# MasatoAkiyama/jama16-retina-replication

Hardware: AMD Instinct MI355X
Metric: train images/sec, Inception-v3 299^2 bs64/GPU (higher is better)
Workload: dtype f32; 1 GPU; Inception-v3 299x299 f32 training, batch 64/GPU, Nesterov lr 3e-3 m 0.9; model=inception_v3, global_batch=64, parallelism=dp1, ranks=1, hip_graph=False, lanes=2, tiles=pinned

## Files before the change

### include/jr.h

```cpp
#ifndef JR_H_
#define JR_H_

#include <stddef.h>
#include <stdint.h>

#ifdef __cplusplus
extern "C" {
#endif

typedef enum jr_status {
  JR_OK = 0,
  JR_ERR_INVALID = -1,
  JR_ERR_HIP = -2,
  JR_ERR_UNSUPPORTED = -3,
  JR_ERR_WORKSPACE = -4,
  JR_ERR_DEVICE = -5
} jr_status;

typedef enum jr_dtype { JR_F32 = 0, JR_BF16 = 1, JR_F32_X8 = 2, JR_F32_X8P = 3, JR_F32_X6H = 4 } jr_dtype;

typedef enum jr_conv_op { JR_CONV_FWD = 0, JR_CONV_BWD_DATA = 1, JR_CONV_BWD_FILTER = 2 } jr_conv_op;

typedef enum jr_head_mode { JR_HEAD_SIGMOID = 0, JR_HEAD_SOFTMAX = 1 } jr_head_mode;

// ... 44 lines not shown
int jr_conv2d_fwd_bn_partials(const jr_conv_desc* d, int dtype, const void* x, const void* w, void* y, void* ws,
                              size_t ws_bytes, void* stream);
int jr_conv2d_bwd_data(const jr_conv_desc* d, int dtype, const void* dy, const void* w, void* dx,
                       int accumulate, void* ws, size_t ws_bytes, void* stream);
int jr_conv2d_bwd_filter(const jr_conv_desc* d, int dtype, const void* x, const void* dy, float* dw,
                         void* ws, size_t ws_bytes, void* stream);

typedef struct jr_wgrad_seg {
  const float* slabs;
  float* dw;
  int32_t m, n, splits, c_in, c_pad, g, block0, blocks;
} jr_wgrad_seg;
int jr_conv2d_wgrad_seg(const jr_conv_desc* d, int dtype, jr_wgrad_seg* seg);
int jr_conv2d_bwd_filter_slabs(const jr_conv_desc* d, int dtype, const void* x, const void* dy, float* slabs,
                               size_t slab_bytes, void* stream);
int jr_wgrad_reduce(const jr_wgrad_seg* segs, int32_t nseg, int32_t total_blocks, void* stream);

int jr_conv2d_autotune(const jr_conv_desc* d, int op, int dtype, const void* a, const void* b, void* c,
                       void* ws, size_t ws_bytes, void* stream);
int jr_conv2d_get_config(const jr_conv_desc* d, int op, int dtype, int phase);
int jr_conv2d_set_config(const jr_conv_desc* d, int op, int dtype, int phase, int cfg);
int jr_conv2d_num_configs(int dtype);
unsigned long long jr_conv2d_config_generation(void);

size_t jr_bn_workspace_size(int64_t m, int32_t c);
typedef struct jr_bn_launch_plan {
  int32_t vec_width, rows_per_chunk, nchunks, single_stage;
  int32_t reduce_grid, finalize_grid, stats_finalize_grid, apply_grid;
  int32_t fold_rows, fold_grid_x, fold_grid_y, reserved;
  int64_t k1_offset, workspace_size;
} jr_bn_launch_plan;
int jr_bn_plan(int dtype, int64_t m, int32_t c, jr_bn_launch_plan* out);
int jr_bn_stats(int dtype, const void* x, int64_t m, int32_t c, float eps, float* mean, float* invstd,
                void* ws, size_t ws_bytes, void* stream);
int jr_bn_relu_apply(int dtype, const void* x, int32_t x_c_off, int32_t x_c_stride, int64_t m, int32_t c,
                     const float* mean, const float* invstd, const float* beta, void* y, int32_t y_c_off,
                     int32_t y_c_stride, void* stream);
typedef struct jr_bn_apply_seg {
  void* y;
  int32_t y_c_off, y_c_stride, c;
  const float* beta;
} jr_bn_apply_seg;
int jr_bn_relu_apply_multi(int dtype, int nseg, const jr_bn_apply_seg* segs, const void* x, int32_t x_c_off,
                           int32_t x_c_stride, int64_t m, int32_t c, const float* mean, const float* invstd,
                           void* stream);
int jr_bn_relu_apply_stats(int dtype, const void* x, int32_t x_c_off, int32_t x_c_stride, int64_t m, int32_t c,
// ... 167 lines not shown
```

### jama16-retina-replication_amd/csrc/jr_common.h

```cpp
#pragma once
#include <hip/hip_runtime.h>
#include <hip/hip_bf16.h>
#include <stdint.h>
#include <cstdlib>
#include <string>

#include "jr_bn_plan.h"
#include "jr_error.h"

namespace jr {

int check_launch(const char* what);

inline hipStream_t as_stream(void* s) { return reinterpret_cast<hipStream_t>(s); }

unsigned* stream_scratch(hipStream_t s, int kind, size_t words);

unsigned* device_error_word(hipStream_t s);

__device__ __forceinline__ int xcd_remap(int orig, int nwg) {
  const int xcd = orig & 7;
  const int q = nwg >> 3, r = nwg & 7;
  const int base = xcd < r ? xcd * (q + 1) : r * (q + 1) + (xcd - r) * q;
  return base + (orig >> 3);
}

__device__ __forceinline__ float bf2f(uint16_t v) {
  return __uint_as_float(static_cast<uint32_t>(v) << 16);
}
__device__ __forceinline__ uint16_t f2bf(float f) {
  __hip_bfloat16 h = __float2bfloat16(f);
  return *reinterpret_cast<uint16_t*>(&h);
}

__device__ __forceinline__ float bn_xhat(float x, float mean, float invstd) {
  return __fmul_rn(__fsub_rn(x, mean), invstd);
}
__device__ __forceinline__ float bn_pre(float x, float mean, float invstd, float beta) {
  return __fadd_rn(bn_xhat(x, mean, invstd), beta);
}

__device__ __forceinline__ void stats_combine8(const float* __restrict__ pm, const float* __restrict__ pq, int P,
                                               int R, int M, float eps, int j, float* mean, float* invstd) {
  const double K = pm[0];
  double sn = 0, sd = 0, sq = 0;
  constexpr int U = 16;
  for (int i0 = j; i0 < P; i0 += kStatsLanes * U) {
    float vm[U], vq[U];
// ... 57 lines not shown
```

### jama16-retina-replication_amd/csrc/jr_conv.hip

```cpp
#include "jr_conv_loop.h"

#include <algorithm>
#include <type_traits>
#include <vector>

namespace jr {

__device__ __forceinline__ uint32_t pk_bf16(float a, float b) {
  const bf16x2 r = {(__bf16)a, (__bf16)b};
  return __builtin_bit_cast(uint32_t, r);
}

__device__ __forceinline__ float sub_f32(float a, float b) {
  float r;
  asm("v_sub_f32 %0, %1, %2" : "=v"(r) : "v"(a), "v"(b));
  return r;
}

__device__ __forceinline__ float lo_bf16_f32(uint32_t u) {
  uint32_t r;
  asm("v_lshlrev_b32 %0, 16, %1" : "=v"(r) : "v"(u));
  return __uint_as_float(r);
}

// ... 70 lines not shown
    }
#pragma unroll
    for (int p = 0; p < 4; ++p) lp[p] = pkrtz_f16(x[2 * p], x[2 * p + 1]);
  }
  typedef uint32_t u32x4 __attribute__((ext_vector_type(4)));
  __device__ __forceinline__ f16x8 h() const { return __builtin_bit_cast(f16x8, (u32x4){hp[0], hp[1], hp[2], hp[3]}); }
  __device__ __forceinline__ f16x8 m() const { return __builtin_bit_cast(f16x8, (u32x4){mp[0], mp[1], mp[2], mp[3]}); }
  __device__ __forceinline__ f16x8 l() const { return __builtin_bit_cast(f16x8, (u32x4){lp[0], lp[1], lp[2], lp[3]}); }
};

template <int OP, int BM, int BN, int WGM, int BK, int NBUF, bool UT, bool X8, int DBG = 0, bool SK = false,
          bool H6 = false>
__global__ void __launch_bounds__(256) k_conv(ConvArgs g) {
  using G = TileGeom<BM, BN, WGM, 4, BK, 4>;
  constexpr int WGN = G::WGN, WM = G::WM, WN = G::WN, TM = G::TM, TN = G::TN;
  constexpr int QPR = G::QPR, RPI = G::RPI, SWZ = G::SWZ, ASZ = G::ASZ, BSZ = G::BSZ;
  constexpr int A_INSTR = G::A_INSTR, B_INSTR = G::B_INSTR, A_PW = G::A_PW, B_PW = G::B_PW;
  constexpr int HALF = BK / 2;
  constexpr bool A_KC = (OP != OP_WGRAD);
  constexpr bool B_KC = (OP == OP_DGRAD);
  constexpr int SMEM = NBUF * (ASZ + BSZ) > 4 * stage_floats<WN>() ? NBUF * (ASZ + BSZ) : 4 * stage_floats<WN>();
  __shared__ __attribute__((aligned(1024))) float smem[SMEM];
  JR_ST(Stamps stamp; stamp.start();)
  member_offsets(g);

  const int tid = threadIdx.x;
  const int lane = tid & 63;
  const int wave = __builtin_amdgcn_readfirstlane(tid >> 6);
  float h_sa = 1.f, h_sb = 1.f, h_one = 1.f;
  if constexpr (H6) {
    asm volatile("" : "+s"(h_one));
    h_sa = __uint_as_float(__builtin_amdgcn_readfirstlane(
        __float_as_uint(pow2_scale(g.a_max ? absmax64(g.a_max, lane) : g.a_bnd))));
    h_sb = __uint_as_float(__builtin_amdgcn_readfirstlane(
        __float_as_uint(pow2_scale(g.b_max ? absmax64(g.b_max, lane) : g.b_bnd))));
  }
  const int wm0 = (wave / WGN) * WM;
  const int wn0 = (wave % WGN) * WN;

  long long sk_it = 0, sk_end = 0;
  const int lb = SK ? xcd_remap(blockIdx.x, gridDim.x) : 0;
  if constexpr (SK) {
    const long long W = (long long)((g.M + BM - 1) / BM) * g.ntn * g.ktiles;
    sk_it = (long long)lb * g.sk_ipb;
    sk_end = sk_it + g.sk_ipb < W ? sk_it + g.sk_ipb : W;
  }
  bool sk_first = true;
  for (;;) {
  int tile, kt0, kt1;
  if constexpr (SK) {
    if (sk_it >= sk_end) break;
    tile = (int)(sk_it / g.ktiles);
    kt0 = (int)(sk_it - (long long)tile * g.ktiles);
    kt1 = (int)(sk_end - sk_it < (long long)(g.ktiles - kt0) ? kt0 + (sk_end - sk_it) : g.ktiles);
    sk_it += kt1 - kt0;
    if (!sk_first) __syncthreads();
  } else {
    tile = xcd_remap(blockIdx.x, gridDim.x);
    kt0 = blockIdx.z * g.kt_per_split;
    kt1 = min(g.ktiles, kt0 + g.kt_per_split);
  }
  const int mt = tile / g.ntn, nt = tile - mt * g.ntn;
  const int m0 = mt * BM, n0 = nt * BN;
  const float* zp = g_zero_page;
  const int cred = OP == OP_FWD ? g.cp : g.cout;
  constexpr bool ut = UT && OP != OP_WGRAD;
  const int wq = OP == OP_WGRAD ? BK / g.wo : 0, wr = OP == OP_WGRAD ? BK - wq * g.wo : 0;
  const int dW0 = OP == OP_WGRAD ? (wq * g.sh * g.w + wr * g.sw) * g.xs : 0;
  const int dW1 = OP == OP_WGRAD ? (g.sh * g.w - g.wo * g.sw) * g.xs : 0;
  const int dW2 = OP == OP_WGRAD ? (g.h * g.w - g.ho * g.sh * g.w) * g.xs : 0;

  const float* a_ptr[A_PW];
  int a_p0[A_PW], a_p1[A_PW], a_p2[A_PW];
  int a_s0[A_PW], a_s1[A_PW], a_s2[A_PW];
  int a_off[A_PW];
#pragma unroll
  for (int i = 0; i < A_PW; ++i) {
    const int j = wave + 4 * i;
    a_ptr[i] = zp;
    a_p0[i] = a_p1[i] = a_p2[i] = 0;
    a_s0[i] = a_s1[i] = a_s2[i] = 0;
    a_off[i] = 0;
// ... 528 lines not shown
    if (rc) return rc;
    hipLaunchKernelGGL(k_stats_finalize, dim3(N, 1, members), dim3(256), 0, s, (const float*)s2,
                       (const float*)(s2 + 2 * (size_t)N * S), S, 0, M, N, S, st->eps, st->mean, st->invstd,
                       (float*)nullptr, pm, st_mb);
  }
  return check_launch("conv stats finalize");
}

static int run_conv1_direct(const jr_conv_desc* d, int dtype, const void* x, const void* w, void* y, void* ws,
                            size_t ws_bytes, hipStream_t s, const StatsReq* st, int members = 1, long long x_mb = 0,
                            long long w_mb = 0, long long y_mb = 0, long long st_mb = 0) {
  int P, R;
  conv1_direct_partials(d, &P, &R);
  const size_t wsm = conv1_direct_ws(d);
  if (st && (!ws || ws_bytes < wsm * members)) return fail(JR_ERR_WORKSPACE, "conv1 direct: workspace too small");
  float* stats = st ? static_cast<float*>(ws) : nullptr;
  launch_conv1_direct(d, dtype, x, w, y, stats, members, x_mb, w_mb, y_mb, (long long)wsm, s);
  int rc = check_launch("conv1 direct");
  if (rc || !st) return rc;
  const long long M = (long long)d->n * d->ho * d->wo;
  return finalize_stats(stats, P, R, (int)M, d->c_out, members, (long long)wsm, st, st_mb, s);
}

template <int OP>
static int run_gemm(int dtype, ConvArgs a, const Plan& p, void* out, void* ws, size_t ws_bytes, hipStream_t s,
                    const StatsReq* st = nullptr, bool defer = false, int members = 1, long long st_mb = 0) {
  if (p.M <= 0 || p.N <= 0) return JR_OK;
  const size_t wsm = members > 1 ? member_ws(dtype, p, st != nullptr) : 0;
  if (members > 1 && (!ws || ws_bytes < wsm * members) && (p.splits > 1 || st))
    return fail(JR_ERR_WORKSPACE, "conv grouped: workspace too small (jr_conv2d_workspace_size_grouped)");
  int sP = 0, sR = 0;
  if (st) {
    stats_geom(dtype, p, &sP, &sR);
    const size_t off = align256(plan_ws(p));
    if (!ws || ws_bytes < off + stats_ws(dtype, p)) return fail(JR_ERR_WORKSPACE, "conv: workspace too small for BN statistics");
    a.stats = reinterpret_cast<float*>(static_cast<char*>(ws) + off);
    a.stats_p = sP;
    a.s_mb = (long long)wsm;
  }
  a.M = p.M; a.N = p.N; a.K = p.K;
  JR_ST(a.dbg = g_dbg_stamps;)
  a.ktiles = p.ktiles;
  a.kt_per_split = p.kt_per_split;
  a.ntn = p.nt;
  a.slab_elems = (long long)p.M * p.N;
  if (p.splits > 1) {
    if (!ws || ws_bytes < plan_ws(p)) return fail(JR_ERR_WORKSPACE, "conv: workspace too small for split-K");
    a.C = static_cast<float*>(ws);
    a.c_mb = (long long)wsm;
  } else {
    a.C = static_cast<float*>(out);
    a.c_mb = a.o_mb;
  }
  dim3 grid(p.mt * p.nt, members, p.splits);
  if (p.sk) {
    if (!ws || ws_bytes < plan_ws(p) + (members > 1 ? (size_t)(members - 1) * wsm : 0))
      return fail(JR_ERR_WORKSPACE, "conv: workspace too small for the stream-K hand-off");
    a.sk_ipb = p.sk_ipb;
    a.sk_part = static_cast<float*>(ws);
    a.sk_mb = (long long)wsm;
    a.sk_flags = stream_scratch(s, 0, (size_t)p.sk_blocks * members);
    if (!a.sk_flags) return fail(JR_ERR_HIP, "conv: stream-K flag words could not be allocated");
    a.sk_fmb = (long long)p.sk_blocks * sizeof(unsigned);
    a.sk_err = device_error_word(s);
    if (!a.sk_err) return fail(JR_ERR_HIP, "conv: no device error word (call jr_init before capturing)");
    grid = dim3(p.sk_blocks, members, 1);
  }
  const CfgEntry& e = cfg_entry(dtype, p.tile);
  switch (e.kernel) {
    case Kernel::HALO:
      a.halo_wp = a.w + a.kw - 1;
      a.halo_nr = (e.t->bm + a.wo - 2) / a.wo + 1 + a.kh - 1;
      launch_conv_halo(e.index, a, grid, s);
      break;
    case Kernel::BF16:
    case Kernel::BF16_WIDE: {
      const TileCfg& t = *e.t;
      int am;
      if (OP == OP_WGRAD) {
        am = t.bk / a.wo < a.ho ? 1 : 2;
      } else {
        const int cred = OP == OP_FWD ? a.cp : a.cout;
        am = cred % t.bk == 0 ? 0 : cred >= t.bk ? 1 : 2;
      }
      const bool wide = e.kernel == Kernel::BF16_WIDE;
      const int np = dtype == JR_F32_X8P ? 3 : 1;
      if (e.sk) launch_conv_bf16_sk(OP, e.index, wide, am, a, grid, s);
      else if (wide) launch_conv_bf16_wide(OP, e.index, am, a, grid, s, np);
      else launch_conv_bf16(OP, e.index, am, a, grid, s, np);
// ... 404 lines not shown
  return autotune(d, op, dtype, a, b, c, ws, ws_bytes, stream, 3);
}

JR_API int jr_conv2d_num_configs(int dtype) { return cfg_count(dtype); }

JR_API int jr_conv2d_debug_time(const jr_conv_desc* d, int cfg, int dbg, const void* x, const void* w, void* y,
                                int reps, float* ms, void* stream) {
  int rc = validate(d, OP_FWD, JR_F32);
  if (rc) return rc;
  const bool x8 = dbg >= 16;
  if (x8) dbg -= 16;
  if (cfg < 0 || cfg >= kNumCfgs || dbg < 0 || dbg > (x8 ? 4 : 3)) return fail(JR_ERR_INVALID, "debug_time: bad cfg/dbg");
  if (dbg > 0 && chan_pad(d->c_in, JR_F32) % kCfgs[cfg].bk != 0)
    return fail(JR_ERR_UNSUPPORTED, "debug_time: variants need c_in % BK == 0");
  ConvArgs a = conv_args(d, OP_FWD, JR_F32, x, w);
  a.C = (float*)y;
  Plan p = plan_for(d, OP_FWD, JR_F32, Phase{}, cfg);
  p.splits = 1; p.kt_per_split = p.ktiles;
  a.M = p.M; a.N = p.N; a.K = p.K; a.ktiles = p.ktiles; a.kt_per_split = p.kt_per_split; a.ntn = p.nt;
  hipStream_t s = as_stream(stream);
  hipEvent_t e0, e1;
  (void)hipEventCreate(&e0);
  (void)hipEventCreate(&e1);
  dim3 grid(p.mt * p.nt, 1, 1);
  (void)hipEventRecord(e0, s);
  for (int r = 0; r < reps; ++r) {
    switch (dbg + (x8 ? 16 : 0)) {
      case 0: launch_op<OP_FWD, 0>(cfg, a, grid, s); break;
      case 1: launch_op<OP_FWD, 1>(cfg, a, grid, s); break;
      case 2: launch_op<OP_FWD, 2>(cfg, a, grid, s); break;
      case 3: launch_op<OP_FWD, 3>(cfg, a, grid, s); break;
      case 16: launch_op<OP_FWD, 0, true>(cfg, a, grid, s); break;
      case 17: launch_op<OP_FWD, 1, true>(cfg, a, grid, s); break;
      case 18: launch_op<OP_FWD, 2, true>(cfg, a, grid, s); break;
      case 19: launch_op<OP_FWD, 3, true>(cfg, a, grid, s); break;
      default: launch_op<OP_FWD, 4, true>(cfg, a, grid, s); break;
    }
  }
  (void)hipEventRecord(e1, s);
  (void)hipEventSynchronize(e1);
  (void)hipEventElapsedTime(ms, e0, e1);
  (void)hipEventDestroy(e0);
  (void)hipEventDestroy(e1);
  return check_launch("debug_time");
}

JR_API int jr_conv2d_set_config(const jr_conv_desc* d, int op, int dtype, int phase, int cfg) {
// ... 22 lines not shown
```

### jama16-retina-replication_amd/csrc/jr_conv_bf16.hip

```cpp
#include "jr_conv_loop.h"

namespace jr {

__device__ __forceinline__ s16x4 lds_tr(const uint16_t* p) {
  return __builtin_amdgcn_ds_read_tr16_b64_v4i16(
      (__attribute__((address_space(3))) s16x4*)(const_cast<uint16_t*>(p)));
}

template <int OP, int BM, int BN, int WGM, int BK, int NBUF, int AM, int NP, int NW, bool SK = false>
__global__ void __launch_bounds__(NW * 64) k_conv_bf16(ConvArgs g) {
  static_assert(NP == 1 || NP == 3, "one bf16 plane, or the h / m / l planes of X8P");
  static_assert(NW == 4 || NW == 8, "4 or 8 waves per block");
  using G = TileGeom<BM, BN, WGM, NW, BK, 8>;
  constexpr int WGN = G::WGN, WM = G::WM, WN = G::WN, TM = G::TM, TN = G::TN;
  constexpr int QPR = G::QPR, RPI = G::RPI, SWZ = G::SWZ, ASZ = G::ASZ, BSZ = G::BSZ;
  constexpr int A_INSTR = G::A_INSTR, B_INSTR = G::B_INSTR, A_PW = G::A_PW, B_PW = G::B_PW;
  constexpr int KSTEPS = BK / 16;
  constexpr bool MC = (OP == OP_WGRAD);
  static_assert(BK % 16 == 0 && QPR <= 8, "BK must be 16..64");
  constexpr int STAGE = NP * (ASZ + BSZ);
  constexpr int SMEM = NBUF * STAGE > 2 * NW * stage_floats<WN>() ? NBUF * STAGE : 2 * NW * stage_floats<WN>();
  static_assert(SMEM * 2 <= 160 * 1024, "LDS budget of one CU");
  __shared__ __attribute__((aligned(1024))) uint16_t smem[SMEM];

  JR_ST(Stamps stamp; stamp.start();)
  member_offsets(g);
  const uint16_t* __restrict__ gA = reinterpret_cast<const uint16_t*>(g.A);
  const uint16_t* __restrict__ gB = reinterpret_cast<const uint16_t*>(g.B);
  const int tid = threadIdx.x;
  const int lane = tid & 63;
  const int wave = __builtin_amdgcn_readfirstlane(tid >> 6);
  const int wm0 = (wave / WGN) * WM;
  const int wn0 = (wave % WGN) * WN;

  long long sk_it = 0, sk_end = 0;
  const int lb = SK ? xcd_remap(blockIdx.x, gridDim.x) : 0;
  if constexpr (SK) {
    const long long W = (long long)((g.M + BM - 1) / BM) * g.ntn * g.ktiles;
    sk_it = (long long)lb * g.sk_ipb;
    sk_end = sk_it + g.sk_ipb < W ? sk_it + g.sk_ipb : W;
  }
  bool sk_first = true;
  for (;;) {
  int tile, kt0, kt1;
  if constexpr (SK) {
    if (sk_it >= sk_end) break;
    tile = (int)(sk_it / g.ktiles);
    kt0 = (int)(sk_it - (long long)tile * g.ktiles);
    kt1 = (int)(sk_end - sk_it < (long long)(g.ktiles - kt0) ? kt0 + (sk_end - sk_it) : g.ktiles);
    sk_it += kt1 - kt0;
    if (!sk_first) __syncthreads();
  } else {
    tile = xcd_remap(blockIdx.x, gridDim.x);
    kt0 = blockIdx.z * g.kt_per_split;
    kt1 = min(g.ktiles, kt0 + g.kt_per_split);
  }
  const int mt = tile / g.ntn, nt = tile - mt * g.ntn;
  const int m0 = mt * BM, n0 = nt * BN;
  unsigned long long zpa = reinterpret_cast<unsigned long long>(g_zero_page);
  asm volatile("" : "+s"(zpa));
  const uint16_t* zp = reinterpret_cast<const uint16_t*>(zpa);
  const int cred = OP == OP_FWD ? g.cp : g.cout;
  const long long psA = NP > 1 ? g.a_ps : 0, psB = NP > 1 ? g.b_ps : 0;
  constexpr bool ut = AM == 0 && OP != OP_WGRAD;

  const int wq = OP == OP_WGRAD ? BK / g.wo : 0, wr = OP == OP_WGRAD ? BK - wq * g.wo : 0;
  constexpr bool inc_a = AM == 1;
  constexpr bool inc_b = OP == OP_DGRAD && AM == 1;
  const int dA0 = OP == OP_WGRAD ? (wq * g.sh * g.w + wr * g.sw) * g.xs : BK;
  const int dA1 = OP == OP_FWD ? BK - g.cp + g.xs
                  : OP == OP_DGRAD ? BK - g.cout - g.ys
                                   : (g.sh * g.w - g.wo * g.sw) * g.xs;
  const int dA2 = OP == OP_FWD ? BK - g.cp + g.xs + (g.w - g.kw) * g.xs
                  : OP == OP_DGRAD ? BK - g.cout + (g.nb - 1 - g.wo) * g.ys
                                   : (g.h * g.w - g.ho * g.sh * g.w) * g.xs;
  const int dB1 = OP == OP_DGRAD ? BK - g.cout + g.sw * g.cin * g.cout : 0;
  const int dB2 = OP == OP_DGRAD ? BK - g.cout + (g.sh * g.kw - g.sw * (g.nb - 1)) * g.cin * g.cout : 0;
// ... 458 lines not shown
```

### jama16-retina-replication_amd/csrc/jr_conv_halo.hip

```cpp
#include "jr_conv_loop.h"

namespace jr {

template <int KH, int KW, int BM, int BN, int WGM, int NBUF, int SLOTS>
__global__ void __launch_bounds__(256) k_conv_halo(ConvArgs g) {
  constexpr int BK = 32;
  constexpr int TAPS = KH * KW;
  using G = WaveTile<BM, BN, WGM, 4>;
  constexpr int WGN = G::WGN, WM = G::WM, WN = G::WN, TM = G::TM, TN = G::TN;
  static_assert(SLOTS % 16 == 0 && (TAPS * BN) % 16 == 0, "images must be whole DMA instructions");
  constexpr int A_INSTR = SLOTS / 16, B_INSTR = TAPS * BN / 16;
  constexpr int A_PW = (A_INSTR + 3) / 4, B_PW = (B_INSTR + 3) / 4;
  constexpr int ASZ = SLOTS * BK, BSZ = TAPS * BN * BK;
  constexpr int STAGE = ASZ + BSZ;
  constexpr int SMEM = NBUF * STAGE > 8 * stage_floats<WN>() ? NBUF * STAGE : 8 * stage_floats<WN>();
  __shared__ __attribute__((aligned(1024))) uint16_t smem[SMEM];
  constexpr int NPIECE = A_PW + B_PW;
  constexpr int per_tile = A_INSTR / 4 + B_INSTR / 4;
  constexpr int KSTEPS = 2 * TAPS;

  member_offsets(g);
  const uint16_t* __restrict__ gA = reinterpret_cast<const uint16_t*>(g.A);
  const uint16_t* __restrict__ gB = reinterpret_cast<const uint16_t*>(g.B);
  const int tid = threadIdx.x;
  const int lane = tid & 63;
  const int wave = __builtin_amdgcn_readfirstlane(tid >> 6);
  const int wm0 = (wave / WGN) * WM;
  const int wn0 = (wave % WGN) * WN;
  const int tile = xcd_remap(blockIdx.x, gridDim.x);
  const int mt = tile / g.ntn, nt = tile - mt * g.ntn;
  const int m0 = mt * BM, n0 = nt * BN;
  const int kt0 = blockIdx.z * g.kt_per_split;
  const int kt1 = min(g.ktiles, kt0 + g.kt_per_split);
  const uint16_t* zp = reinterpret_cast<const uint16_t*>(g_zero_page);
  const int WP = g.halo_wp;
  const int gr0 = m0 / g.wo;
  const int glo = gr0 - g.ph;
  const int nslots = g.halo_nr * WP;
  const int grows = g.n * g.h;

  const uint16_t* a_ptr[A_PW];
#pragma unroll
  for (int i = 0; i < A_PW; ++i) {
    const int j = wave + 4 * i;
    a_ptr[i] = nullptr;
    if (A_INSTR % 4 != 0 && j >= A_INSTR) continue;
    const int e = j * 64 + lane;
    const int s = e >> 2, q = (e & 3) ^ ((s >> 2) & 3);
    if (s < nslots) {
      const int sr = s / WP, sc = s - sr * WP;
      const int G = glo + sr, iw = sc - g.pw;
      if ((unsigned)G < (unsigned)grows && (unsigned)iw < (unsigned)g.w)
        a_ptr[i] = gA + (((long long)G * g.w + iw) * g.xs + g.xo + q * 8);
    }
  }
// ... 141 lines not shown
```

### jama16-retina-replication_amd/csrc/jr_conv_impl.h

```cpp
#pragma once
#include "jr_common.h"
#include "jr_conv_plan.h"

#include <type_traits>

namespace jr {

typedef float f32x16 __attribute__((ext_vector_type(16)));

static __device__ __attribute__((aligned(64))) float g_zero_page[16];

struct ConvArgs {
  const float* A;
  const float* B;
  float* C;
  int M, N, K;
  int n, h, w, cin, cp, cout, kh, kw, sh, sw, ph, pw, ho, wo;
  int xo, xs, yo, ys;
  int c_off, c_stride;
  int accumulate;
  int ktiles, kt_per_split, ntn;
  long long slab_elems;
  float* stats;
  int stats_p;
  int py, px, r0, c0, na, nb, ey, ex, hc, wc;
  long long a_ps, b_ps;
  int halo_nr, halo_wp;
  unsigned long long* dbg;
  long long a_mb, b_mb, c_mb, s_mb, o_mb;
  long long sk_ipb, sk_mb, sk_fmb;
  unsigned* sk_flags;
  float* sk_part;
  unsigned* sk_err;
  const float* a_max;
  const float* b_max;
  float a_bnd, b_bnd;
};

__device__ __forceinline__ float absmax64(const float* p, int lane) {
  float v = p[lane];
#pragma unroll
  for (int o = 32; o >= 1; o >>= 1) v = fmaxf(v, __shfl_xor(v, o, 64));
  return v;
}

__device__ __forceinline__ float pow2_scale(float m) {
  const unsigned b = __float_as_uint(m);
  const int eb = (int)((b >> 23) & 0xffu);
  if (!(m > 0.f) || eb == 255) return 1.f;
  const int biased = min(268 - eb, 227);
  return __uint_as_float((unsigned)biased << 23);
}

__device__ __forceinline__ void member_offsets(ConvArgs& g) {
  if (gridDim.y > 1) {
    const long long m = blockIdx.y;
    g.A = reinterpret_cast<const float*>(reinterpret_cast<const char*>(g.A) + m * g.a_mb);
    g.B = reinterpret_cast<const float*>(reinterpret_cast<const char*>(g.B) + m * g.b_mb);
    g.C = reinterpret_cast<float*>(reinterpret_cast<char*>(g.C) + m * g.c_mb);
    if (g.stats) g.stats = reinterpret_cast<float*>(reinterpret_cast<char*>(g.stats) + m * g.s_mb);
    if (g.a_max) g.a_max += 64 * m;
    if (g.b_max) g.b_max += 64 * m;
    if (g.sk_flags) {
      g.sk_flags = reinterpret_cast<unsigned*>(reinterpret_cast<char*>(g.sk_flags) + m * g.sk_fmb);
      g.sk_part = reinterpret_cast<float*>(reinterpret_cast<char*>(g.sk_part) + m * g.sk_mb);
    }
  }
}

#ifdef JR_STAMPS
struct Stamps {
  unsigned long long r0, c0, cp, cl, w;
  __device__ __forceinline__ void start() {
    r0 = __builtin_amdgcn_s_memrealtime();
    c0 = __builtin_amdgcn_s_memtime();
    w = 0;
  }
  __device__ __forceinline__ void prologue() { cp = __builtin_amdgcn_s_memtime(); }
  __device__ __forceinline__ void loop() { cl = __builtin_amdgcn_s_memtime(); }
  __device__ __forceinline__ unsigned long long now() { return __builtin_amdgcn_s_memtime(); }
  __device__ __forceinline__ void end(unsigned long long* dbg) {
    const unsigned long long ce = __builtin_amdgcn_s_memtime(), re = __builtin_amdgcn_s_memrealtime();
    if (dbg == nullptr || threadIdx.x != 0) return;
    unsigned long long* o = dbg + 8ull * (blockIdx.z * gridDim.x + blockIdx.x);
    o[0] = r0; o[1] = re; o[2] = cp - c0; o[3] = cl - cp; o[4] = ce - cl; o[5] = w;
    o[6] = __builtin_amdgcn_s_getreg((31 << 11) | 4);
    o[7] = __builtin_amdgcn_s_getreg((3 << 11) | 20);
  }
};
#define JR_ST(x) x
#else
#define JR_ST(x)
#endif

__device__ __forceinline__ long long dgrad_pix(const ConvArgs& g, int m) {
  const int hw = g.hc * g.wc;
  const int b = m / hw, rem = m - b * hw;
  const int u = rem / g.wc, v = rem - u * g.wc;
  return ((long long)b * g.h + g.sh * u + g.py) * g.w + g.sw * v + g.px;
}

template <int OP>
__device__ __forceinline__ long long out_row(const ConvArgs& g, int m) {
  if constexpr (OP == OP_FWD) {
    return (long long)m * g.c_stride + g.c_off;
  } else if constexpr (OP == OP_DGRAD) {
    return dgrad_pix(g, m) * g.c_stride + g.c_off;
// ... 155 lines not shown
  }
  sk_sum_pieces<TM, TN, NW>(g, acc, wave, lane, owner, npieces, st == 2);
  return true;
}

__device__ __forceinline__ bool sk_cut(const ConvArgs& g, int tile, int kt0, int kt1, int* owner, int* npieces,
                                       int* kind) {
  if (kt0 == 0 && kt1 == g.ktiles) return false;
  const long long t0 = (long long)tile * g.ktiles;
  *owner = (int)(t0 / g.sk_ipb);
  *npieces = (int)((t0 + g.ktiles - 1) / g.sk_ipb) - *owner + 1;
  *kind = kt0 == 0 ? 1 : 0;
  return true;
}


template <int WN> constexpr int stage_floats() { return 32 * (WN + 8); }

template <int OP, int WM, int TM, int TN, bool BF16K>
__device__ __forceinline__ void conv_epilogue(const ConvArgs& g, f32x16 (&acc)[TM][TN], float* stage, int mw0,
                                              int nw0, int lane) {
  constexpr int WN = TN * 32, S = WN + 8, LPR = WN / 8, NIT = 32 * LPR / 64;
  static_assert((32 * LPR) % 64 == 0, "stage read-back must be whole wave-instructions");
  const bool split = gridDim.z > 1;
  const bool bout = BF16K && OP != OP_WGRAD && !split;
  const int l31 = lane & 31, lh = lane >> 5;
  auto row_of = [&](int r) { return (r & 3) + 8 * (r >> 2) + 4 * lh; };
  if constexpr (OP == OP_FWD) {
    if (g.stats != nullptr && !split) {
      const int P = g.stats_p;
      const int pidx = mw0 / WM;
      const int nv = min(max(g.M - mw0, 0), WM);
#pragma unroll
      for (int j = 0; j < TN; ++j) {
        float s = 0.f;
#pragma unroll
        for (int i = 0; i < TM; ++i)
#pragma unroll
          for (int r = 0; r < 16; ++r) {
            float v = acc[i][j][r];
            if (bout) { v = bf2f(f2bf(v)); acc[i][j][r] = v; }
            s += (mw0 + i * 32 + row_of(r) < g.M) ? v : 0.f;
          }
        s += __shfl_xor(s, 32, 64);
        const float mu = nv > 0 ? s / (float)nv : 0.f;
        float q = 0.f;
#pragma unroll
        for (int i = 0; i < TM; ++i)
#pragma unroll
          for (int r = 0; r < 16; ++r) {
            const float d = acc[i][j][r] - mu;
            q += (mw0 + i * 32 + row_of(r) < g.M) ? d * d : 0.f;
          }
        q += __shfl_xor(q, 32, 64);
        const int n = nw0 + j * 32 + l31;
        if (lh == 0 && n < g.N) {
          g.stats[(long long)n * P + pidx] = mu;
          g.stats[(long long)(g.N + n) * P + pidx] = q;
        }
      }
    }
  }
  float* C = split ? g.C + (long long)blockIdx.z * g.slab_elems : g.C;
#pragma unroll
  for (int i = 0; i < TM; ++i) {
#pragma unroll
    for (int j = 0; j < TN; ++j)
#pragma unroll
      for (int r = 0; r < 16; ++r) stage[row_of(r) * S + j * 32 + l31] = acc[i][j][r];
    asm volatile("s_waitcnt lgkmcnt(0)" ::: "memory");
    constexpr int CH = NIT % 4 == 0 ? 4 : NIT % 3 == 0 ? 3 : NIT % 2 == 0 ? 2 : 1;
#pragma unroll
    for (int i0 = 0; i0 < NIT; i0 += CH) {
      float v[CH][8];
      long long off[CH];
      bool ok[CH];
#pragma unroll
      for (int k = 0; k < CH; ++k) {
        const int e = (i0 + k) * 64 + lane;
        const int row = e / LPR, c8 = (e - row * LPR) * 8;
        const float4 v0 = *reinterpret_cast<const float4*>(stage + row * S + c8);
        const float4 v1 = *reinterpret_cast<const float4*>(stage + row * S + c8 + 4);
        v[k][0] = v0.x; v[k][1] = v0.y; v[k][2] = v0.z; v[k][3] = v0.w;
        v[k][4] = v1.x; v[k][5] = v1.y; v[k][6] = v1.z; v[k][7] = v1.w;
        const int m = mw0 + i * 32 + row, n = nw0 + c8;
        ok[k] = m < g.M && n < g.N;
// ... 233 lines not shown
```

### jama16-retina-replication_amd/csrc/jr_conv_plan.cpp

```cpp
#include "jr_conv_plan.h"

#include <algorithm>
#include <cstdlib>
#include <map>
#include <mutex>
#include <vector>

namespace jr {

struct CfgSpace {
  std::vector<CfgEntry> ids;
  int std;
};

static CfgSpace build_space(int dtype) {
  CfgSpace s;
  auto tiles = [&](Kernel k, const TileCfg* t, int n, bool sk) {
    for (int i = 0; i < n; ++i) s.ids.push_back(CfgEntry{k, i, sk, t + i, nullptr});
  };
  switch (dtype) {
    case JR_F32:
      tiles(Kernel::F32_MFMA, kCfgs, kNumCfgs, false);
      s.std = kNumCfgs;
      break;
    case JR_F32_X8:
// ... 295 lines not shown
  std::lock_guard<std::mutex> lk(c.mu);
  auto it = c.tuned.find(k);
  return it != c.tuned.end() ? it->second : -1;
}

void tune_set(const TuneKey& k, int cfg) {
  TuneCache& c = tune_cache();
  std::lock_guard<std::mutex> lk(c.mu);
  auto it = c.tuned.find(k);
  if (cfg < 0) {
    if (it != c.tuned.end()) { c.tuned.erase(it); ++c.gen; }
  } else if (it == c.tuned.end() || it->second != cfg) {
    c.tuned[k] = cfg;
    ++c.gen;
  }
}

unsigned long long tune_generation() {
  TuneCache& c = tune_cache();
  std::lock_guard<std::mutex> lk(c.mu);
  return c.gen;
}

}
```

### jama16-retina-replication_amd/csrc/jr_conv_plan.h

```cpp
#pragma once
#include <array>
#include <cstddef>

#include "jr_error.h"

namespace jr {

enum { OP_FWD = 0, OP_DGRAD = 1, OP_WGRAD = 2 };

inline size_t align256(size_t b) { return (b + 255) / 256 * 256; }

#ifndef JR_STATS_CHUNK
#define JR_STATS_CHUNK 4096
#endif
constexpr int kStatsChunk = JR_STATS_CHUNK;

struct TileCfg {
  int bm, bn, wgm, bk, nbuf;
  double eff;
  int nw = 4;
};

static constexpr TileCfg kCfgs[] = {
    {128, 128, 2, 16, 3, 1.00},
    {128, 128, 2, 32, 2, 1.00},
    {256, 64, 4, 16, 3, 1.00},
// ... 166 lines not shown
```

### jama16-retina-replication_amd/jr/_ffi.py

```python
from __future__ import annotations

import ctypes
import os
from ctypes import (POINTER, Structure, c_char_p, c_double, c_float, c_int, c_int32, c_int64,
                    c_size_t, c_uint8, c_void_p)

_HERE = os.path.dirname(os.path.abspath(__file__))
LIB_PATH = os.environ.get("JR_LIB", os.path.join(_HERE, "libjr.so"))

JR_OK = 0
JR_ERR_INVALID, JR_ERR_HIP, JR_ERR_UNSUPPORTED, JR_ERR_WORKSPACE = -1, -2, -3, -4
JR_ERR_DEVICE = -5
JR_F32 = 0
JR_BF16 = 1
JR_F32_X8 = 2
JR_F32_X8P = 3
JR_F32_X6H = 4
JR_CONV_FWD, JR_CONV_BWD_DATA, JR_CONV_BWD_FILTER = 0, 1, 2
JR_HEAD_SIGMOID, JR_HEAD_SOFTMAX = 0, 1


class JRError(RuntimeError):

    def __init__(self, fn: str, status: int, msg: str):
# ... 79 lines not shown
    "jr_conv2d_fwd_bn_partials": (c_int, [POINTER(ConvDesc), c_int, c_void_p, c_void_p, c_void_p, c_void_p, c_size_t,
                                          c_void_p]),
    "jr_bn_relu_apply_stats": (c_int, [c_int, c_void_p, c_int32, c_int32, c_int64, c_int32, c_void_p, c_int32, c_int32,
                                       c_int32, c_int32, c_float, c_void_p, c_void_p, c_void_p, c_void_p, c_int32,
                                       c_int32, c_void_p]),
    "jr_conv2d_workspace_size_grouped": (c_size_t, [POINTER(ConvDesc), c_int, c_int]),
    "jr_conv2d_fwd_bn_stats_grouped": (c_int, [POINTER(ConvDesc), c_int, c_int, c_void_p, c_int64, c_void_p, c_int64,
                                               c_void_p, c_int64, c_float, c_void_p, c_void_p, c_int64, c_void_p,
                                               c_size_t, c_void_p]),
    "jr_conv2d_bwd_data": (c_int, [POINTER(ConvDesc), c_int, c_void_p, c_void_p, c_void_p, c_int,
                                   c_void_p, c_size_t, c_void_p]),
    "jr_conv2d_bwd_filter": (c_int, [POINTER(ConvDesc), c_int, c_void_p, c_void_p, c_void_p,
                                     c_void_p, c_size_t, c_void_p]),
    "jr_conv2d_wgrad_seg": (c_int, [POINTER(ConvDesc), c_int, POINTER(WgradSeg)]),
    "jr_conv2d_bwd_filter_slabs": (c_int, [POINTER(ConvDesc), c_int, c_void_p, c_void_p, c_void_p, c_size_t,
                                           c_void_p]),
    "jr_wgrad_reduce": (c_int, [c_void_p, c_int32, c_int32, c_void_p]),
    "jr_conv2d_autotune": (c_int, [POINTER(ConvDesc), c_int, c_int, c_void_p, c_void_p, c_void_p,
                                   c_void_p, c_size_t, c_void_p]),
    "jr_conv2d_get_config": (c_int, [POINTER(ConvDesc), c_int, c_int, c_int]),
    "jr_conv2d_set_config": (c_int, [POINTER(ConvDesc), c_int, c_int, c_int, c_int]),
    "jr_conv2d_config_generation": (ctypes.c_ulonglong, []),
    "jr_conv2d_num_configs": (c_int, [c_int]),
    "jr_conv_weights_bf16_tiles": (c_int32, [c_int32, c_int32, c_int32, c_int32]),
    "jr_conv_weights_bf16": (c_int, [c_void_p, c_int32, c_int32, c_int32, c_int32, c_void_p, c_void_p,
                                     c_void_p]),
    "jr_conv_weights_bf16_multi": (c_int, [c_void_p, c_int32, c_int32, c_void_p, c_void_p, c_void_p,
                                           c_void_p]),
    "jr_conv_weights_x8p": (c_int, [c_void_p, c_int32, c_int32, c_int32, c_int32, c_void_p, c_void_p,
                                    c_void_p]),
    "jr_conv_weights_x8p_multi": (c_int, [c_void_p, c_int32, c_int32, c_void_p, c_void_p, c_void_p,
                                          c_void_p]),
    "jr_split_x8p": (c_int, [c_void_p, c_int64, c_int32, c_int32, c_int32, c_void_p, c_int32, c_int32, c_int32,
                             c_int64, c_void_p]),
    "jr_comm_unique_id": (c_int, [c_void_p]),
    "jr_comm_init": (c_int, [c_int, c_int, c_void_p, c_int, c_void_p]),
    "jr_comm_init_file": (c_int, [c_int, c_int, c_char_p, c_char_p, c_int, c_int, c_void_p]),
    "jr_allreduce_sum": (c_int, [c_void_p, c_void_p, c_size_t, c_int, c_void_p]),
    "jr_comm_rank": (c_int, [c_void_p]),
    "jr_comm_world": (c_int, [c_void_p]),
    "jr_comm_destroy": (c_int, [c_void_p]),
    "jr_bn_workspace_size": (c_size_t, [c_int64, c_int32]),
    "jr_bn_plan": (c_int, [c_int, c_int64, c_int32, POINTER(BnLaunchPlan)]),
    "jr_bn_relu_bwd_batch_workspace_size": (c_size_t, [c_int32, c_void_p]),
    "jr_bn_relu_apply_multi": (c_int, [c_int, c_int, c_void_p, c_void_p, c_int32, c_int32, c_int64, c_int32,
                                       c_void_p, c_void_p, c_void_p]),
# ... 177 lines not shown
```

### jama16-retina-replication_amd/jr/engine.py

```python
from __future__ import annotations

import ctypes
import dataclasses
import json
import os
from typing import Callable, Dict, List, Optional, Tuple

import numpy as np
import torch

from . import _ffi
from .inception import BN_EPS, Graph, PoolNode, build_inception_v3
from .init import init_params
from .lanes import Build, Call, Lanes, node_lanes, schedule
from .plan import ConvUnit, bn_batch_groups, bn_moving_segments, build_plan

DTYPES = {"f32": _ffi.JR_F32, "bf16": _ffi.JR_BF16}


_PINNED = None


def fusable_pools(g: Graph, plan) -> Dict[int, int]:
    out = {}
# ... 155 lines not shown
            self.labels[:y.numel()].copy_(y, non_blocking=True)

    def _check_images(self, images, B: int) -> None:
        ib = self.g.bufs[self.g.input_buf]
        if B > self.batch or B <= 0:
            raise ValueError(f"batch {B} outside 1..{self.batch}")
        if tuple(images.shape[1:]) != (ib.h, ib.w, ib.c):
            raise ValueError(f"images must be [B,{ib.h},{ib.w},{ib.c}] NHWC, got {tuple(images.shape)}")

    def _alloc_bn_moving(self) -> None:
        self.moving = self._t(self.members * self.stats_ms)
        self.frozen = self._t(self.members * self.stats_ms)
        self._bn_tables: Dict[int, tuple] = {}
        self._reset_bn_moving()
        self.frozen_source = None
        self.updates = 0

    def _reset_bn_moving(self, var: float = 1.0) -> None:
        host = np.zeros((self.members, self.stats_ms), np.float32)
        off = 0
        for u in self.cunits:
            host[:, off + u.cout:off + 2 * u.cout] = var
            off += 2 * u.cout
        with torch.cuda.stream(self.stream):
            self.moving.copy_(torch.from_numpy(host.reshape(-1)).to(self.device))

    def _bn_table(self, B: int) -> tuple:
        if B not in self._bn_tables:
            segs = [_ffi.BnMovingSeg(so, mo, rows, c, 0) for so, mo, rows, c in bn_moving_segments(self.cunits, B)]
            self._bn_tables[B] = (self._table(_ffi.BnMovingSeg, segs), len(segs), max(u.cout for u in self.cunits))
        return self._bn_tables[B]

    def _bn_update_args(self, B: int, momentum: float, s) -> tuple:
        table, nseg, max_c = self._bn_table(B)
        return (table.data_ptr(), nseg, max_c, self.members, self.stats.data_ptr(), self.stats_ms,
                self.moving.data_ptr(), self.stats_ms, float(momentum), BN_EPS, s)

    def _bn_layers(self):
        off = 0
        for u in self.cunits:
            for n, co in zip(u.members, u.col_off):
                yield n, off + co, off + u.cout + co
            off += 2 * u.cout

    def _bn_moving_get(self) -> List[dict]:
        self.synchronize()
# ... 892 lines not shown
```

Before: 3029 images/sec.

## Flatten conv grid and apply XCD remap across tiles, members and splits

Conv kernels now launch a 1-D grid by default and decode each block's tile, member and split index through one global XCD remap, replacing the per-tile remap on a 3-D grid. The goal is to place blocks that share operands (same member or split) on the same XCD so they reuse its L2. Decoding uses a magic-number divide, the split slab offset moves into the block setup, and an env var or API call can restore the old order. The cost is a little extra index arithmetic per block, and it may scatter tiles that previously shared data within an XCD.

```diff
diff --git a/include/jr.h b/include/jr.h
--- a/include/jr.h
+++ b/include/jr.h
@@ -90,6 +90,9 @@
 int jr_conv2d_set_config(const jr_conv_desc* d, int op, int dtype, int phase, int cfg);
 int jr_conv2d_num_configs(int dtype);
 unsigned long long jr_conv2d_config_generation(void);
+int jr_conv2d_get_block_order(void);
+int jr_conv2d_set_block_order(int order);
+int jr_conv2d_block_map(int order, int ntiles, int members, int splits, int32_t* out);
 
 size_t jr_bn_workspace_size(int64_t m, int32_t c);
 typedef struct jr_bn_launch_plan {
diff --git a/jama16-retina-replication_amd/csrc/jr_block_order.h b/jama16-retina-replication_amd/csrc/jr_block_order.h
--- /dev/null
+++ b/jama16-retina-replication_amd/csrc/jr_block_order.h
@@ -0,0 +1,44 @@
+#pragma once
+
+#if defined(__HIP__)
+#define JR_HD __attribute__((host)) __attribute__((device)) inline __attribute__((always_inline))
+#else
+#define JR_HD inline
+#endif
+
+namespace jr {
+
+JR_HD int xcd_remap(int orig, int nwg) {
+  const int xcd = orig & 7;
+  const int q = nwg >> 3, r = nwg & 7;
+  const int base = xcd < r ? xcd * (q + 1) : r * (q + 1) + (xcd - r) * q;
+  return base + (orig >> 3);
+}
+
+struct BlockPos {
+  int tile, member, split;
+};
+
+JR_HD BlockPos conv_block_pos(int order, int id, int ntiles, int members, int splits, unsigned magic) {
+  const int l = order ? xcd_remap(id, ntiles * members * splits) : id;
+  int ms = 0;
+  if (members * splits > 1)
+    ms = magic ? (int)(((unsigned long long)(unsigned)l * magic) >> 32) : ntiles == 1 ? l : (int)((unsigned)l / (unsigned)ntiles);
+  const int t = l - ms * ntiles;
+  const int s = members > 1 ? (int)((unsigned)ms / (unsigned)members) : ms;
+  return BlockPos{order ? t : xcd_remap(t, ntiles), ms - s * members, s};
+}
+
+JR_HD unsigned div_magic(int d, long long n) {
+  if (d <= 1 || (unsigned long long)n * (unsigned)d > (1ull << 32)) return 0;
+  return (unsigned)(((1ull << 32) + (unsigned)d - 1) / (unsigned)d);
+}
+
+JR_HD BlockPos conv_block_pos(int order, int id, int ntiles, int members, int splits) {
+  return conv_block_pos(order, id, ntiles, members, splits, div_magic(ntiles, (long long)ntiles * members * splits));
+}
+
+int conv_block_order();
+int set_conv_block_order(int order);
+
+}
diff --git a/jama16-retina-replication_amd/csrc/jr_common.h b/jama16-retina-replication_amd/csrc/jr_common.h
--- a/jama16-retina-replication_amd/csrc/jr_common.h
+++ b/jama16-retina-replication_amd/csrc/jr_common.h
@@ -5,6 +5,7 @@
 #include <cstdlib>
 #include <string>
 
+#include "jr_block_order.h"
 #include "jr_bn_plan.h"
 #include "jr_error.h"
 
@@ -18,12 +19,6 @@
 
 unsigned* device_error_word(hipStream_t s);
 
-__device__ __forceinline__ int xcd_remap(int orig, int nwg) {
-  const int xcd = orig & 7;
-  const int q = nwg >> 3, r = nwg & 7;
-  const int base = xcd < r ? xcd * (q + 1) : r * (q + 1) + (xcd - r) * q;
-  return base + (orig >> 3);
-}
 
 __device__ __forceinline__ float bf2f(uint16_t v) {
   return __uint_as_float(static_cast<uint32_t>(v) << 16);
diff --git a/jama16-retina-replication_amd/csrc/jr_conv.hip b/jama16-retina-replication_amd/csrc/jr_conv.hip
--- a/jama16-retina-replication_amd/csrc/jr_conv.hip
+++ b/jama16-retina-replication_amd/csrc/jr_conv.hip
@@ -116,7 +116,8 @@
   constexpr int SMEM = NBUF * (ASZ + BSZ) > 4 * stage_floats<WN>() ? NBUF * (ASZ + BSZ) : 4 * stage_floats<WN>();
   __shared__ __attribute__((aligned(1024))) float smem[SMEM];
   JR_ST(Stamps stamp; stamp.start();)
-  member_offsets(g);
+  const BlockPos bp = conv_block<SK>(g);
+  block_offsets(g, bp);
 
   const int tid = threadIdx.x;
   const int lane = tid & 63;
@@ -150,8 +151,8 @@
     sk_it += kt1 - kt0;
     if (!sk_first) __syncthreads();
   } else {
-    tile = xcd_remap(blockIdx.x, gridDim.x);
-    kt0 = blockIdx.z * g.kt_per_split;
+    tile = bp.tile;
+    kt0 = bp.split * g.kt_per_split;
     kt1 = min(g.ktiles, kt0 + g.kt_per_split);
   }
   const int mt = tile / g.ntn, nt = tile - mt * g.ntn;
@@ -726,6 +727,13 @@
   return finalize_stats(stats, P, R, (int)M, d->c_out, members, (long long)wsm, st, st_mb, s);
 }
 
+static dim3 conv_grid(ConvArgs& a, int tiles, int members, int splits) {
+  a.b_tiles = tiles; a.b_members = members; a.b_splits = splits;
+  a.b_order = conv_block_order();
+  a.b_magic = div_magic(tiles, (long long)tiles * members * splits);
+  return a.b_order ? dim3(tiles * members * splits) : dim3(tiles, members, splits);
+}
+
 template <int OP>
 static int run_gemm(int dtype, ConvArgs a, const Plan& p, void* out, void* ws, size_t ws_bytes, hipStream_t s,
                     const StatsReq* st = nullptr, bool defer = false, int members = 1, long long st_mb = 0) {
@@ -756,7 +764,8 @@
     a.C = static_cast<float*>(out);
     a.c_mb = a.o_mb;
   }
-  dim3 grid(p.mt * p.nt, members, p.splits);
+  if ((long long)p.mt * p.nt * members * p.splits > 0x7fffffffLL) return fail(JR_ERR_UNSUPPORTED, "conv: too many blocks");
+  dim3 grid = conv_grid(a, p.mt * p.nt, members, p.splits);
   if (p.sk) {
     if (!ws || ws_bytes < plan_ws(p) + (members > 1 ? (size_t)(members - 1) * wsm : 0))
       return fail(JR_ERR_WORKSPACE, "conv: workspace too small for the stream-K hand-off");
@@ -769,6 +778,7 @@
     a.sk_err = device_error_word(s);
     if (!a.sk_err) return fail(JR_ERR_HIP, "conv: no device error word (call jr_init before capturing)");
     grid = dim3(p.sk_blocks, members, 1);
+    a.b_tiles = p.sk_blocks; a.b_members = members; a.b_splits = 1; a.b_order = 0;
   }
   const CfgEntry& e = cfg_entry(dtype, p.tile);
   switch (e.kernel) {
@@ -1219,7 +1229,7 @@
   hipEvent_t e0, e1;
   (void)hipEventCreate(&e0);
   (void)hipEventCreate(&e1);
-  dim3 grid(p.mt * p.nt, 1, 1);
+  const dim3 grid = conv_grid(a, p.mt * p.nt, 1, 1);
   (void)hipEventRecord(e0, s);
   for (int r = 0; r < reps; ++r) {
     switch (dbg + (x8 ? 16 : 0)) {
diff --git a/jama16-retina-replication_amd/csrc/jr_conv_bf16.hip b/jama16-retina-replication_amd/csrc/jr_conv_bf16.hip
--- a/jama16-retina-replication_amd/csrc/jr_conv_bf16.hip
+++ b/jama16-retina-replication_amd/csrc/jr_conv_bf16.hip
@@ -24,7 +24,8 @@
   __shared__ __attribute__((aligned(1024))) uint16_t smem[SMEM];
 
   JR_ST(Stamps stamp; stamp.start();)
-  member_offsets(g);
+  const BlockPos bp = conv_block<SK>(g);
+  block_offsets(g, bp);
   const uint16_t* __restrict__ gA = reinterpret_cast<const uint16_t*>(g.A);
   const uint16_t* __restrict__ gB = reinterpret_cast<const uint16_t*>(g.B);
   const int tid = threadIdx.x;
@@ -51,8 +52,8 @@
     sk_it += kt1 - kt0;
     if (!sk_first) __syncthreads();
   } else {
-    tile = xcd_remap(blockIdx.x, gridDim.x);
-    kt0 = blockIdx.z * g.kt_per_split;
+    tile = bp.tile;
+    kt0 = bp.split * g.kt_per_split;
     kt1 = min(g.ktiles, kt0 + g.kt_per_split);
   }
   const int mt = tile / g.ntn, nt = tile - mt * g.ntn;
diff --git a/jama16-retina-replication_amd/csrc/jr_conv_halo.hip b/jama16-retina-replication_amd/csrc/jr_conv_halo.hip
--- a/jama16-retina-replication_amd/csrc/jr_conv_halo.hip
+++ b/jama16-retina-replication_amd/csrc/jr_conv_halo.hip
@@ -19,7 +19,8 @@
   constexpr int per_tile = A_INSTR / 4 + B_INSTR / 4;
   constexpr int KSTEPS = 2 * TAPS;
 
-  member_offsets(g);
+  const BlockPos bp = conv_block<false>(g);
+  block_offsets(g, bp);
   const uint16_t* __restrict__ gA = reinterpret_cast<const uint16_t*>(g.A);
   const uint16_t* __restrict__ gB = reinterpret_cast<const uint16_t*>(g.B);
   const int tid = threadIdx.x;
@@ -27,10 +28,10 @@
   const int wave = __builtin_amdgcn_readfirstlane(tid >> 6);
   const int wm0 = (wave / WGN) * WM;
   const int wn0 = (wave % WGN) * WN;
-  const int tile = xcd_remap(blockIdx.x, gridDim.x);
+  const int tile = bp.tile;
   const int mt = tile / g.ntn, nt = tile - mt * g.ntn;
   const int m0 = mt * BM, n0 = nt * BN;
-  const int kt0 = blockIdx.z * g.kt_per_split;
+  const int kt0 = bp.split * g.kt_per_split;
   const int kt1 = min(g.ktiles, kt0 + g.kt_per_split);
   const uint16_t* zp = reinterpret_cast<const uint16_t*>(g_zero_page);
   const int WP = g.halo_wp;
diff --git a/jama16-retina-replication_amd/csrc/jr_conv_impl.h b/jama16-retina-replication_amd/csrc/jr_conv_impl.h
--- a/jama16-retina-replication_amd/csrc/jr_conv_impl.h
+++ b/jama16-retina-replication_amd/csrc/jr_conv_impl.h
@@ -28,6 +28,8 @@
   int halo_nr, halo_wp;
   unsigned long long* dbg;
   long long a_mb, b_mb, c_mb, s_mb, o_mb;
+  int b_tiles, b_members, b_splits, b_order;
+  unsigned b_magic;
   long long sk_ipb, sk_mb, sk_fmb;
   unsigned* sk_flags;
   float* sk_part;
@@ -52,9 +54,18 @@
   return __uint_as_float((unsigned)biased << 23);
 }
 
-__device__ __forceinline__ void member_offsets(ConvArgs& g) {
-  if (gridDim.y > 1) {
-    const long long m = blockIdx.y;
+template <bool SK>
+__device__ __forceinline__ BlockPos conv_block(const ConvArgs& g) {
+  if constexpr (SK) return BlockPos{0, (int)blockIdx.y, 0};
+  const int id = blockIdx.x + g.b_tiles * (blockIdx.y + g.b_members * blockIdx.z);
+  const BlockPos p = conv_block_pos(g.b_order, id, g.b_tiles, g.b_members, g.b_splits, g.b_magic);
+  return BlockPos{__builtin_amdgcn_readfirstlane(p.tile), __builtin_amdgcn_readfirstlane(p.member),
+                  __builtin_amdgcn_readfirstlane(p.split)};
+}
+
+__device__ __forceinline__ void block_offsets(ConvArgs& g, const BlockPos& p) {
+  if (g.b_members > 1) {
+    const long long m = p.member;
     g.A = reinterpret_cast<const float*>(reinterpret_cast<const char*>(g.A) + m * g.a_mb);
     g.B = reinterpret_cast<const float*>(reinterpret_cast<const char*>(g.B) + m * g.b_mb);
     g.C = reinterpret_cast<float*>(reinterpret_cast<char*>(g.C) + m * g.c_mb);
@@ -66,6 +77,7 @@
       g.sk_part = reinterpret_cast<float*>(reinterpret_cast<char*>(g.sk_part) + m * g.sk_mb);
     }
   }
+  if (g.b_splits > 1) g.C += (long long)p.split * g.slab_elems;
 }
 
 #ifdef JR_STAMPS
@@ -82,7 +94,7 @@
   __device__ __forceinline__ void end(unsigned long long* dbg) {
     const unsigned long long ce = __builtin_amdgcn_s_memtime(), re = __builtin_amdgcn_s_memrealtime();
     if (dbg == nullptr || threadIdx.x != 0) return;
-    unsigned long long* o = dbg + 8ull * (blockIdx.z * gridDim.x + blockIdx.x);
+    unsigned long long* o = dbg + 8ull * (blockIdx.x + gridDim.x * (blockIdx.y + gridDim.y * blockIdx.z));
     o[0] = r0; o[1] = re; o[2] = cp - c0; o[3] = cl - cp; o[4] = ce - cl; o[5] = w;
     o[6] = __builtin_amdgcn_s_getreg((31 << 11) | 4);
     o[7] = __builtin_amdgcn_s_getreg((3 << 11) | 20);
@@ -284,7 +296,7 @@
                                               int nw0, int lane) {
   constexpr int WN = TN * 32, S = WN + 8, LPR = WN / 8, NIT = 32 * LPR / 64;
   static_assert((32 * LPR) % 64 == 0, "stage read-back must be whole wave-instructions");
-  const bool split = gridDim.z > 1;
+  const bool split = g.b_splits > 1;
   const bool bout = BF16K && OP != OP_WGRAD && !split;
   const int l31 = lane & 31, lh = lane >> 5;
   auto row_of = [&](int r) { return (r & 3) + 8 * (r >> 2) + 4 * lh; };
@@ -323,7 +335,7 @@
       }
     }
   }
-  float* C = split ? g.C + (long long)blockIdx.z * g.slab_elems : g.C;
+  float* C = g.C;
 #pragma unroll
   for (int i = 0; i < TM; ++i) {
 #pragma unroll
diff --git a/jama16-retina-replication_amd/csrc/jr_conv_plan.cpp b/jama16-retina-replication_amd/csrc/jr_conv_plan.cpp
--- a/jama16-retina-replication_amd/csrc/jr_conv_plan.cpp
+++ b/jama16-retina-replication_amd/csrc/jr_conv_plan.cpp
@@ -1,6 +1,7 @@
 #include "jr_conv_plan.h"
 
 #include <algorithm>
+#include <atomic>
 #include <cstdlib>
 #include <map>
 #include <mutex>
@@ -342,4 +343,43 @@
   return c.gen;
 }
 
-}
+namespace {
+std::atomic<int>& block_order_setting() {
+  static std::atomic<int> v = [] {
+    const char* e = std::getenv("JR_CONV_BLOCK_ORDER");
+    return e && e[0] == '0' && e[1] == 0 ? 0 : 1;
+  }();
+  return v;
+}
+}
+
+int conv_block_order() { return block_order_setting().load(std::memory_order_relaxed); }
+
+int set_conv_block_order(int order) {
+  if (order != 0 && order != 1) return -1;
+  return block_order_setting().exchange(order, std::memory_order_relaxed);
+}
+
+}
+
+JR_API int jr_conv2d_get_block_order(void) { return jr::conv_block_order(); }
+
+JR_API int jr_conv2d_set_block_order(int order) {
+  const int prev = jr::set_conv_block_order(order);
+  if (prev < 0) jr::set_error("conv set_block_order: order must be 0 or 1");
+  return prev;
+}
+
+JR_API int jr_conv2d_block_map(int order, int ntiles, int members, int splits, int32_t* out) {
+  if ((order != 0 && order != 1) || ntiles < 1 || members < 1 || splits < 1 || !out ||
+      (long long)ntiles * members * splits > 0x7fffffffLL)
+    return jr::fail(JR_ERR_INVALID, "conv block_map: bad order, launch shape or output");
+  const int total = ntiles * members * splits;
+  for (int id = 0; id < total; ++id) {
+    const jr::BlockPos p = jr::conv_block_pos(order, id, ntiles, members, splits);
+    out[3 * id] = p.tile;
+    out[3 * id + 1] = p.member;
+    out[3 * id + 2] = p.split;
+  }
+  return JR_OK;
+}
diff --git a/jama16-retina-replication_amd/csrc/jr_conv_plan.h b/jama16-retina-replication_amd/csrc/jr_conv_plan.h
--- a/jama16-retina-replication_amd/csrc/jr_conv_plan.h
+++ b/jama16-retina-replication_amd/csrc/jr_conv_plan.h
@@ -2,6 +2,7 @@
 #include <array>
 #include <cstddef>
 
+#include "jr_block_order.h"
 #include "jr_error.h"
 
 namespace jr {
diff --git a/jama16-retina-replication_amd/jr/_ffi.py b/jama16-retina-replication_amd/jr/_ffi.py
--- a/jama16-retina-replication_amd/jr/_ffi.py
+++ b/jama16-retina-replication_amd/jr/_ffi.py
@@ -125,6 +125,9 @@
     "jr_conv2d_set_config": (c_int, [POINTER(ConvDesc), c_int, c_int, c_int, c_int]),
     "jr_conv2d_config_generation": (ctypes.c_ulonglong, []),
     "jr_conv2d_num_configs": (c_int, [c_int]),
+    "jr_conv2d_get_block_order": (c_int, []),
+    "jr_conv2d_set_block_order": (c_int, [c_int]),
+    "jr_conv2d_block_map": (c_int, [c_int, c_int, c_int, c_int, c_void_p]),
     "jr_conv_weights_bf16_tiles": (c_int32, [c_int32, c_int32, c_int32, c_int32]),
     "jr_conv_weights_bf16": (c_int, [c_void_p, c_int32, c_int32, c_int32, c_int32, c_void_p, c_void_p,
                                      c_void_p]),
diff --git a/jama16-retina-replication_amd/jr/engine.py b/jama16-retina-replication_amd/jr/engine.py
--- a/jama16-retina-replication_amd/jr/engine.py
+++ b/jama16-retina-replication_amd/jr/engine.py
@@ -201,6 +201,7 @@
         for u in self.cunits:
             host[:, off + u.cout:off + 2 * u.cout] = var
             off += 2 * u.cout
+        self.stream.wait_stream(torch.cuda.current_stream(self.device))
         with torch.cuda.stream(self.stream):
             self.moving.copy_(torch.from_numpy(host.reshape(-1)).to(self.device))
 
```

After: 3048 images/sec, median of 6. No clear change (+0.6%).
